# hvasbath/beat

Measured on AMD Instinct MI355X. Metric: SMC chain-steps/s (FFI seismic gfstacking 400 patches x 64 targets x 4096 samples), higher is better.
Workload: dtype f64

## Files before the change

### beat_amd/csrc/capi.cpp

```cpp
#include "kernels.hpp"

using namespace beatamd;

namespace {

int dev_alloc_copy(beatamd_ctx *ctx, const void *src, size_t bytes, void **dst)
{
    void *d = nullptr;
    hipError_t e = hipMalloc(&d, bytes ? bytes : 8);
    if (e != hipSuccess) {
        (void)hipGetLastError();
        set_error("hipMalloc(%zu bytes) failed: %s", bytes, hipGetErrorString(e));
        return BEATAMD_ENOMEM;
    }
    if (src && bytes) {
        e = hipMemcpyAsync(d, src, bytes, hipMemcpyDefault, ctx->stream);
        if (e == hipSuccess) e = hipStreamSynchronize(ctx->stream);
        if (e != hipSuccess) {
            (void)hipFree(d);
            set_error("hipMemcpy(%zu bytes) failed: %s", bytes, hipGetErrorString(e));
            return BEATAMD_EHIP;
        }
    }
    *dst = d;
// ... 21 lines not shown

#define ENTER(ctx)                                                    \
    BA_CHECK((ctx) != nullptr, BEATAMD_EINVAL, "ctx is NULL");        \
    BA_HIP(hipSetDevice((ctx)->device))

int wset_quad(beatamd_ctx *ctx, const WeightSet &w, int64_t C, const double *X, int64_t xs_c,
              int64_t xs_d, double *quad)
{
    if (w.kind == BEATAMD_W_SCALAR)
        return launch_scalar_quad(ctx, C, w.nd, w.M, X, xs_c, xs_d, w.w, quad);
    if (w.band >= 0 && w.wb && GfKnobs::get(gf_knobs(ctx).qf_band, 1) != 0)
        return launch_quadform_banded(ctx, w.wb, w.band, w.M, w.nd, C, X, xs_c, xs_d, quad, w.nd);
    QuadformCall q;
    q.A = w.w;
    q.a_stride = w.M * w.M;
    q.M = w.M;
    q.nd = w.nd;
    q.C = C;
    q.X = X;
    q.xs_c = xs_c;
    q.xs_d = xs_d;
    q.upper_tri = w.upper_tri;
    q.quad = quad;
    q.q_stride = w.nd;
    return launch_quadform(ctx, q);
}

struct LikeTail {
    LikeGroups grp;
    const int32_t *chain_bad = nullptr;
};

int ffi_logp_device(beatamd_ctx *ctx, FfiModel &m, int64_t C, const double *Q, double *LL,
                    LikeTail *tail = nullptr)
{
    const int64_t nllk = m.nllk();
    const int64_t np = m.layout.nparams;
    void *p = nullptr;
    LikeGroups grp;
    int64_t col = 0;

    ChainVec slips[4];
    for (int v = 0; v < m.layout.nvar; v++) slips[v] = ChainVec{Q, np, m.layout.slip_off[v]};

    int32_t *chain_bad = nullptr;
    if (!m.wavemaps.empty()) {
        BA_TRY(ctx->get_scratch(SL_CHAINBAD, (size_t)C * sizeof(int32_t), &p));
        chain_bad = (int32_t *)p;
        BA_HIP(hipMemsetAsync(chain_bad, 0, (size_t)C * sizeof(int32_t), ctx->stream));
    }

    if (!m.wavemaps.empty()) {
        BA_TRY(ctx->get_scratch(SL_ST0, (size_t)C * m.P * sizeof(double), &p));
        double *st0 = (double *)p;
        BA_TRY(launch_sweep_model(ctx, m, Q, C, st0, chain_bad));
        for (auto &wm : m.wavemaps) {
            WeightSet *ws = get_obj(ctx->wsets, wm.wset);
            BA_CHECK(ws, BEATAMD_EINVAL, "wavemap refers to a destroyed weight set");
            GfStackCall k;
            k.nvar = m.layout.nvar;
            for (int v = 0; v < k.nvar; v++) {
                k.libs[v] = get_obj(ctx->seislibs, wm.libs[v]);
                BA_CHECK(k.libs[v] && k.libs[v]->g, BEATAMD_EINVAL,
                         "wavemap refers to a destroyed / empty GF library");
                k.slips[v] = slips[v];
            }
            k.durations = ChainVec{Q, np, m.layout.durations_off};
            k.st.starttimes0 = st0;
            k.st.Q = Q;
            k.st.nparams = np;
            k.order_key[0] = ChainVec{Q, np, m.layout.nuc_strike_off};
            k.order_key[1] = ChainVec{Q, np, m.layout.nuc_dip_off};
            k.st.shift_off = wm.shift_off;
            k.st.nslot = wm.nslot; k.st.tslot = wm.tslot; k.st.slot_shift_off = wm.slot_shift_off;
            k.st.chain_bad = chain_bad;
            k.interp = wm.interp;
            k.f32 = wm.f32;
            k.C = C;
            k.data = wm.data;
            BA_TRY(ctx->get_scratch(SL_QUAD, (size_t)C * wm.T * sizeof(double), &p));
            double *quad = (double *)p;
            if (ws->kind == BEATAMD_W_SCALAR) {
                k.mode = GF_RESID_SCALAR;
                k.wscalar = ws->w;
                k.quad = quad;
                BA_TRY(launch_gfstack(ctx, k));
            } else if (ws->band == 1 && ws->wb && ws->M == wm.N && ws->nd == wm.T &&
                       GfKnobs::get(gf_knobs(ctx).qf_band, 1) != 0) {
                k.mode = GF_RESID_BAND1;
                k.band_w = ws->wb;
                k.quad = quad;
                BA_TRY(ctx->get_scratch(SL_RESID, (size_t)C * wm.T * wm.N * sizeof(double), &p));
                k.out = (double *)p;
                BA_TRY(launch_gfstack(ctx, k));
            } else {
                k.mode = GF_RESID_STORE;
                BA_TRY(ctx->get_scratch(SL_RESID, (size_t)C * wm.T * wm.N * sizeof(double), &p));
                k.out = (double *)p;
                BA_TRY(launch_gfstack(ctx, k));
                BA_TRY(wset_quad(ctx, *ws, C, k.out, wm.T * wm.N, wm.N, quad));
            }
            BA_TRY(launch_mvn_finish(ctx, C, wm.T, wm.N, quad, ws->slog, HpSrc{Q, np, wm.hp_off},
                                     LL + col, nllk));
            col += wm.T;
        }
        grp.end[grp.n++] = (int32_t)col;
    }
    if (m.has_geo) {
// ... 896 lines not shown
                double *z = (double *)p, *rs = nullptr;
                if (draw->df > 0) {
                    BA_TRY(ctx->get_scratch(SL_ROWSCALE, (size_t)C * 8, &p));
                    rs = (double *)p;
                }
                BA_TRY(launch_philox_normal(ctx, z, C, K, draw->seed, draw->step, draw->first_chain));
                BA_TRY(launch_philox_chain(ctx, C, draw->seed, draw->step, draw->first_chain, draw->df, lu, rs));
                GemmCall g;
                g.A = z; g.lda = K;
                g.B = (const double *)d_f; g.ldb = np; g.b_kn = 1;
                g.O = de; g.ldo = np;
                g.M = C; g.N = np; g.K = K;
                g.row_scale = rs;
                g.timer = "proposal";
                BA_TRY(launch_gemm_f64(ctx, g));
            } else {
                BA_TRY(launch_philox_univariate(ctx, de, C, np, draw->kind, (const double *)d_f, draw->seed,
                                                draw->step, draw->first_chain));
                BA_TRY(launch_philox_chain(ctx, C, draw->seed, draw->step, draw->first_chain, 0, lu, nullptr));
            }
            BA_TRY(launch_propose(ctx, C, np, (const double *)d_q0, de, (const double *)d_sc,
                                  (const double *)d_lo, (const double *)d_up, qprop, inb));
        }
        advance = true;
    } else {
        BA_TRY(stage_in(ctx, SL_IN1, delta, (size_t)C * np * 8, &d_de));
        BA_TRY(stage_in(ctx, SL_IN5, log_u, (size_t)C * 8, &d_lu));
        BA_TRY(launch_propose(ctx, C, np, (const double *)d_q0, (const double *)d_de,
                              (const double *)d_sc, (const double *)d_lo, (const double *)d_up, qprop,
                              inb));
    }
    LikeTail tail;
    const bool fold = nllk * 8 <= 48 * 1024;
    BA_TRY(ffi_logp_device(ctx, *m, C, qprop, lprop, fold ? &tail : nullptr));
    BA_TRY(launch_accept(ctx, C, np, nllk, (double *)d_q0, (double *)d_l0, qprop, lprop, inb,
                         (const double *)d_lu, beta, (const double *)d_be, (int32_t *)d_acc,
                         fold ? &tail.grp : nullptr, tail.chain_bad, acc_sum, n_acc, advance));
    return finish_out(ctx, recs, 3);
}

int beatamd_ffi_astep_batch(beatamd_ctx *ctx, int32_t model_id, int64_t C, double *Q0, double *L0,
                            const double *delta, const double *scaling, const double *lower,
                            const double *upper, const double *log_u, double beta,
                            int32_t *accepted)
{
    BA_CHECK(ctx != nullptr, BEATAMD_EINVAL, "ctx is NULL");
    return astep_impl(ctx, model_id, C, Q0, L0, delta, scaling, lower, upper, log_u, beta, nullptr,
                      accepted);
}

int beatamd_ffi_astep_batch_betas(beatamd_ctx *ctx, int32_t model_id, int64_t C, double *Q0,
                                  double *L0, const double *delta, const double *scaling,
                                  const double *lower, const double *upper, const double *log_u,
                                  const double *betas, int32_t *accepted)
{
    BA_CHECK(ctx != nullptr && betas != nullptr, BEATAMD_EINVAL, "ffi_astep_betas: NULL argument");
    return astep_impl(ctx, model_id, C, Q0, L0, delta, scaling, lower, upper, log_u, 1.0, betas,
                      accepted);
}

int beatamd_ffi_mstep_batch(beatamd_ctx *ctx, int32_t model_id, int64_t C, double *Q0, double *L0,
                            const double *factor, int64_t K, int32_t kind, int32_t df, uint64_t seed,
                            uint32_t step, int64_t first_chain, const double *scaling, const double *lower,
                            const double *upper, double beta, const double *betas, int32_t *accepted,
                            int32_t *accepted_sum, int64_t *n_accepted)
{
    BA_CHECK(ctx != nullptr, BEATAMD_EINVAL, "ctx is NULL");
// ... 551 lines not shown
```

### beat_amd/csrc/ctx.cpp

```cpp
#include "ctx.hpp"

#include <cstdlib>

namespace beatamd {

static thread_local char g_err[1024] = "";

void set_error(const char *fmt, ...)
{
    va_list ap;
    va_start(ap, fmt);
    vsnprintf(g_err, sizeof(g_err), fmt, ap);
    va_end(ap);
}

int DevBuf::reserve(size_t bytes)
{
    if (bytes <= cap) return BEATAMD_OK;
    size_t want = bytes + bytes / 4;
    if (p) {
        BA_HIP(hipDeviceSynchronize());
        BA_HIP(hipFree(p));
        p = nullptr;
        cap = 0;
// ... 147 lines not shown
        }
        if (st & ST_BAD_HYPO) {
            set_error("nucleation index outside the patch grid");
            return BEATAMD_EINVAL;
        }
        if (st & ST_BAD_COV) {
            set_error("Sample covariances contains Inf or NaN! Please try reducing the upper and lower bounds "
                      "of hyper parameters!");
            return BEATAMD_EBADCOV;
        }
        if (st & ST_NOT_PSD) {
            set_error("Matrix is not positive definite");
            return BEATAMD_ENOTPSD;
        }
        if (st & ST_BAD_SCALE) {
            set_error("PoissonProposal: a step width outside (0, 500] (or NaN): the draws of that parameter are NaN");
            return BEATAMD_EINVAL;
        }
    }
    return BEATAMD_OK;
}

namespace beatamd {

void GfKnobs::read_env()
{
    auto rd = [](const char *name) { const char *e = getenv(name); return e ? atoi(e) : KNOB_UNSET; };
    gf_kernel = rd("BEATAMD_GF_KERNEL"); gs_cg = rd("BEATAMD_GS_CG"); gs_ws = rd("BEATAMD_GS_WS"); gs_dma = rd("BEATAMD_GS_DMA");
    gs_nt = rd("BEATAMD_GS_NT"); ws_map = rd("BEATAMD_WS_MAP"); gs_pair = rd("BEATAMD_GS_PAIR"); gs_nthint = rd("BEATAMD_GS_NTHINT");
    gs_order = rd("BEATAMD_GS_ORDER"); gs_fit = rd("BEATAMD_GS_FIT"); gs_win = rd("BEATAMD_GS_WIN"); gf_tinv = rd("BEATAMD_GF_TINV");
    gs_tune = rd("BEATAMD_GS_TUNE"); gf_order = rd("BEATAMD_GF_ORDER"); gf_cgroup = rd("BEATAMD_GF_CGROUP"); gs_ml = rd("BEATAMD_GS_ML");
    gc_global = rd("BEATAMD_GC_GLOBAL"); gc_sort = rd("BEATAMD_GC_SORT"); gc_keys = rd("BEATAMD_GC_KEYS"); gc_bands = rd("BEATAMD_GC_BANDS"); gr_cap = rd("BEATAMD_GR_CAP");
    gr_pass_alloc = rd("BEATAMD_GR_PASS_ALLOC"); gr_var = rd("BEATAMD_GR_VAR"); sweep_v1 = rd("BEATAMD_SWEEP_V1"); qf_band = rd("BEATAMD_QF_BAND"); qf_fuse = rd("BEATAMD_QF_FUSE"); gf_split = rd("BEATAMD_GF_SPLIT"); gm_wave = rd("BEATAMD_GM_WAVE");
}

const GfKnobs &gf_knobs(beatamd_ctx *ctx)
{
    if (ctx->knobs_live) ctx->knobs.read_env();
    return ctx->knobs;
}

}

extern "C" {

const char *beatamd_last_error(void) { return g_err; }

int beatamd_version(void) { return BEATAMD_VERSION; }

int beatamd_ctx_create(int device, beatamd_ctx **out)
{
    BA_CHECK(out != nullptr, BEATAMD_EINVAL, "ctx_create: out is NULL");
    int ndev = 0;
    hipError_t e = hipGetDeviceCount(&ndev);
    if (e != hipSuccess || ndev == 0) {
        (void)hipGetLastError();
        set_error("no HIP device available (%s)", hipGetErrorString(e));
        return BEATAMD_EHIP;
    }
    BA_CHECK(device >= 0 && device < ndev, BEATAMD_EINVAL, "device %d out of range [0,%d)", device,
             ndev);
    BA_HIP(hipSetDevice(device));
    beatamd_ctx *c = new beatamd_ctx();
    c->device = device;
    BA_HIP(hipStreamCreateWithFlags(&c->own_stream, hipStreamNonBlocking));
    c->stream = c->own_stream;
// ... 159 lines not shown
```

### beat_amd/csrc/ctx.hpp

```cpp
#pragma once
#include <hip/hip_runtime.h>

#include <cstdarg>
#include <cstdint>
#include <cstdio>
#include <cstring>
#include <map>
#include <memory>
#include <string>
#include <vector>

#include "../../include/beat_amd.h"

namespace beatamd {

void set_error(const char *fmt, ...);

#define BA_HIP(expr)                                                                         \
    do {                                                                                     \
        hipError_t e_ = (expr);                                                              \
        if (e_ != hipSuccess) {                                                              \
            beatamd::set_error("%s:%d: %s -> %s", __FILE__, __LINE__, #expr,                 \
                               hipGetErrorString(e_));                                       \
            return BEATAMD_EHIP;                                                             \
// ... 80 lines not shown
struct GeomSources {
    int nsrc = 0;
    int32_t *kind = nullptr;
    int64_t *poff = nullptr;
    double *pfix = nullptr;
    double *east = nullptr, *north = nullptr, *los = nullptr;
    int64_t Nobs = 0;
    double nu = 0.25;
};

struct FfiModel {
    beatamd_ffi_layout layout;
    int32_t nsub = 0;
    std::vector<int32_t> ndip, nstrike, patch_off;
    std::vector<double> patch_size;
    int64_t P = 0;
    int32_t *d_ndip = nullptr, *d_nstrike = nullptr, *d_patch_off = nullptr;
    double *d_patch_size = nullptr;
    std::vector<Wavemap> wavemaps;
    bool has_geo = false;
    Geodetic geo;
    bool geo_is_geometry = false;
    GeomSources geom;
    int32_t lap = -1;
    int64_t nllk() const;
};

constexpr int KNOB_UNSET = -2147483647;
struct GfKnobs {
    int gf_kernel = KNOB_UNSET, gs_cg = KNOB_UNSET, gs_ws = KNOB_UNSET, gs_dma = KNOB_UNSET, gs_nt = KNOB_UNSET,
        ws_map = KNOB_UNSET, gs_pair = KNOB_UNSET, gs_nthint = KNOB_UNSET, gs_order = KNOB_UNSET, gs_fit = KNOB_UNSET,
        gs_win = KNOB_UNSET, gf_tinv = KNOB_UNSET, gs_tune = KNOB_UNSET, gf_order = KNOB_UNSET, gf_cgroup = KNOB_UNSET,
        gs_ml = KNOB_UNSET, gc_global = KNOB_UNSET, gc_sort = KNOB_UNSET, gc_keys = KNOB_UNSET, gc_bands = KNOB_UNSET, gr_cap = KNOB_UNSET,
        gr_pass_alloc = KNOB_UNSET, gr_var = KNOB_UNSET, sweep_v1 = KNOB_UNSET, qf_band = KNOB_UNSET, qf_fuse = KNOB_UNSET, gf_split = KNOB_UNSET, gm_wave = KNOB_UNSET;
    void read_env();
    static int get(int v, int dflt) { return v == KNOB_UNSET ? dflt : v; }
    static bool is(int v, int x) { return v != KNOB_UNSET && v == x; }
    static bool set(int v) { return v != KNOB_UNSET; }
};

struct KTimer {
    double total_ms = 0;
    int64_t n = 0;
    std::vector<std::pair<hipEvent_t, hipEvent_t>> pending;
};

}

struct beatamd_ctx {
    int device = 0;
    hipStream_t stream = nullptr, own_stream = nullptr;
    bool timing = false;
    std::map<std::string, beatamd::KTimer> timers;
    std::vector<hipEvent_t> event_pool;
    int *d_status = nullptr;
    std::vector<beatamd::DevBuf> scratch;
    std::vector<std::unique_ptr<beatamd::SeisLib>> seislibs;
    std::vector<std::unique_ptr<beatamd::GeoLib>> geolibs;
    std::vector<std::unique_ptr<beatamd::WeightSet>> wsets;
    std::vector<std::unique_ptr<beatamd::Laplacian>> laps;
    std::vector<std::unique_ptr<beatamd::FfiModel>> models;
    int num_cu = 256;
    char last_gf_kernel[96] = "";
    int64_t gs_ngtp = 0, gs_N = 0;
    double gs_trep = 1;
    int gs_nvar = 1;
    bool gs_has_passes = false;
// ... 19 lines not shown

namespace beatamd {

bool is_device_ptr(const void *p);
const GfKnobs &gf_knobs(beatamd_ctx *ctx);

struct Arg {
    beatamd_ctx *ctx;
    void *host = nullptr;
    void *dev = nullptr;
    size_t bytes = 0;
    bool out = false;
};

int stage_in(beatamd_ctx *ctx, int slot, const void *p, size_t bytes, const void **dev);
int stage_out(beatamd_ctx *ctx, int slot, void *p, size_t bytes, void **dev, Arg *rec,
              bool preload = false);
int finish_out(beatamd_ctx *ctx, Arg *recs, int n);

struct ScopedTimer {
    beatamd_ctx *c;
    const char *n;
    ScopedTimer(beatamd_ctx *ctx, const char *name) : c(ctx), n(name) { c->time_begin(n); }
    ~ScopedTimer() { c->time_end(n); }
};

enum Slot : int {
    SL_IN0 = 0, SL_IN1, SL_IN2, SL_IN3, SL_IN4, SL_IN5, SL_IN6, SL_IN7,
    SL_OUT0, SL_OUT1, SL_OUT2,
    SL_ROWOFF, SL_WEIGHTS, SL_ST0, SL_RESID, SL_PARTIAL, SL_PARTIAL2, SL_QUAD, SL_MU, SL_SLIPS,
    SL_QPROP, SL_LPROP, SL_MISC, SL_GS_UROWS, SL_GS_UCOUNT, SL_GS_SLOT, SL_GS_W, SL_GS_UMAX, SL_GS_USLOT,
    SL_CHAINBAD, SL_Z, SL_ROWSCALE, SL_CUM, SL_STAGE2, SL_WHITEN,
    SL_CHOL_A, SL_CHOL_X, SL_CHOL_D, SL_CHOL_T, SL_CHOL_L,
    SL_GC_ORDER, SL_GS_ORDER, SL_GC_STREAM, SL_GC_HDR, SL_GC_META, SL_DELTA, SL_LOGU, SL_EDGES, SL_TSLOT, SL_SPLIT, SL_COUNT
};

}
```

### beat_amd/csrc/gfshared.hip

```cpp
#include "kernels.hpp"

namespace beatamd {

constexpr int GS_NT_MAX = 64;
constexpr int GS_NTHINT_DEFAULT = 1;
constexpr int GS_WS_DEFAULT = 1;

struct GroupTabArgs {
    int nrow, nvar, CG;
    int64_t C, T, P, DS;
    const uint32_t *rowoff;
    const double *fac;
    ChainVec slips[4];
    int ucap, ustride;
    uint32_t *urows;
    uint32_t *uent;
    int nissue;
    int windowed;
    int depth;
    uint32_t *ucount;
    uint32_t *umax;
    uint16_t *slot;
    double *w;
    int64_t w_var_stride;
// ... 933 lines not shown
    const int64_t w_var_bytes = a.w_var_stride * 8;
    auto tab_slot = [&](int p) { return slot_base + (uint32_t)p * slot_step; };
    auto tab_w = [&](int p, int iv) {
        return w_base + (uint32_t)p * w_step + (nvar == 1 ? (int64_t)0 : (int64_t)iv * w_var_bytes);
    };
    auto fetch_tabs = [&](const char *ps, const char *pw) {
        asm("global_load_ushort %0, %1, %2" : "=v"(sl_n) : "v"(voff_s), "s"(ps));
        uint32_t voff_w;
        asm("v_lshlrev_b32 %1, 2, %2\n\t"
            "global_load_dwordx2 %0, %1, %3" : "=v"(wl_n), "=&v"(voff_w) : "v"(voff_s), "s"(pw));
    };
    auto row_address = [&](uint32_t base) {
        uint32_t x;
        asm("s_waitcnt vmcnt(0)\n\t"
            "v_lshl_add_u32 %0, %1, 6, %1\n\t"
            "v_lshl_add_u32 %0, %0, 3, %2" : "=&v"(x) : "v"(sl_n), "s"(base), "v"(wl_n));
        return x;
    };
    auto landed_weight = [&](uint32_t after) {
        double x;
        asm("v_mov_b64 %0, %1" : "=v"(x) : "v"(wl_n), "v"(after));
        return x;
    };
    static_assert(GS_PITCH == 65, "row_address multiplies by 65");
    constexpr int NG8 = GS_NT / 8;
    static_assert(NG8 == 8, "the read schedule below is written for 64-sample tiles");
    double ya[8], yb[8];
    int p1 = 0, iv1 = 0;
    advance(p1, iv1);
    int gbuf = 0;
    const int ring = NB * bufsz;
    double w;
    uint32_t xs;
    fetch_tabs(tab_slot(0), tab_w(0, 0));
    xs = row_address(lds0);
    w = landed_weight(xs);
    __builtin_amdgcn_sched_barrier(0);
    __builtin_amdgcn_s_barrier();
    __builtin_amdgcn_sched_barrier(0);
    lds_rd8_b64<0>(ya, xs, -1);
    lds_rd8_b64<64>(yb, xs, -1);
    __builtin_amdgcn_sched_barrier(0);
    fetch_tabs(tab_slot(p1), tab_w(p1, iv1));
    advance(p1, iv1);
    const char *ps_run = tab_slot(p1), *pw_run = tab_w(p1, iv1);
    int iv_run = iv1;
    const int64_t dw_next = (nvar == 1) ? (int64_t)w_step : w_var_bytes;
    const int64_t dw_wrap = (int64_t)w_step - (int64_t)(nvar - 1) * w_var_bytes;
#pragma clang loop unroll(disable)
    for (int s = 0; s < nsteps; s++) {
        int gnext = gbuf + bufsz;
        if (gnext == ring) gnext = 0;
        __builtin_amdgcn_sched_barrier(0);
#define BA_FMA8 \
    "v_fmac_f64 %0, %8, %16\n\tv_fmac_f64 %1, %9, %16\n\tv_fmac_f64 %2, %10, %16\n\tv_fmac_f64 %3, %11, %16\n\t" \
    "v_fmac_f64 %4, %12, %16\n\tv_fmac_f64 %5, %13, %16\n\tv_fmac_f64 %6, %14, %16\n\tv_fmac_f64 %7, %15, %16\n\t"
#define BA_RD8(OFF) \
    "ds_read_b64 %8, %17 offset:" #OFF "\n\tds_read_b64 %9, %17 offset:" #OFF "+8\n\t" \
    "ds_read_b64 %10, %17 offset:" #OFF "+16\n\tds_read_b64 %11, %17 offset:" #OFF "+24\n\t" \
    "ds_read_b64 %12, %17 offset:" #OFF "+32\n\tds_read_b64 %13, %17 offset:" #OFF "+40\n\t" \
    "ds_read_b64 %14, %17 offset:" #OFF "+48\n\tds_read_b64 %15, %17 offset:" #OFF "+56"
#define BA_ACC8(G) \
    "+v"(acc[G * 8]), "+v"(acc[G * 8 + 1]), "+v"(acc[G * 8 + 2]), "+v"(acc[G * 8 + 3]), "+v"(acc[G * 8 + 4]), \
        "+v"(acc[G * 8 + 5]), "+v"(acc[G * 8 + 6]), "+v"(acc[G * 8 + 7])
#define BA_Y8(Y) "+v"(Y[0]), "+v"(Y[1]), "+v"(Y[2]), "+v"(Y[3]), "+v"(Y[4]), "+v"(Y[5]), "+v"(Y[6]), "+v"(Y[7])
#define BA_FMA4A \
// ... 30 lines not shown
        asm(BA_FMA8
            "v_mov_b64 %16, %18\n\t" BA_RD8(64)
            : BA_ACC8(7), BA_Y8(yb), "+v"(w) : "v"(xs_n), "v"(wl_n));
        xs = xs_n;
        __builtin_amdgcn_sched_barrier(0);
#undef BA_GROUP
#undef BA_RD4B
#undef BA_RD4A
#undef BA_FMA4B
#undef BA_FMA4A
#undef BA_Y8
#undef BA_ACC8
#undef BA_RD8
#undef BA_FMA8
        fetch_tabs(ps_run, pw_run);
        {
            uint32_t ds;
            int64_t dw;
            asm("s_add_i32 %0, %0, 1\n\t"
                "s_cmp_eq_u32 %0, %3\n\t"
                "s_cselect_b32 %0, 0, %0\n\t"
                "s_cselect_b32 %1, %4, 0\n\t"
                "s_cselect_b64 %2, %5, %6"
                : "+s"(iv_run), "=&s"(ds), "=&s"(dw) : "s"(nvar), "s"(slot_step), "s"(dw_wrap), "s"(dw_next) : "scc");
            ps_run += ds;
            pw_run += dw;
        }
    }
    asm volatile("s_waitcnt vmcnt(0) lgkmcnt(0)"
                 : "+v"(ya[0]), "+v"(ya[1]), "+v"(ya[2]), "+v"(ya[3]), "+v"(ya[4]), "+v"(ya[5]), "+v"(ya[6]),
                   "+v"(ya[7]), "+v"(yb[0]), "+v"(yb[1]), "+v"(yb[2]), "+v"(yb[3]), "+v"(yb[4]), "+v"(yb[5]),
                   "+v"(yb[6]), "+v"(yb[7]), "+v"(sl_n), "+v"(wl_n));
    __builtin_amdgcn_sched_barrier(0);

    const bool live = (c < a.C);
    const int nvalid = (int)min((int64_t)GS_NT, N - n0);
    if (MODE == GF_STORE_SYN) {
        if (live) {
            double *o = a.out + (c * a.T + t) * N + n0;
#pragma unroll
            for (int i = 0; i < GS_NT; i++)
                if (i < nvalid) o[i] = acc[i];
        }
        return;
    }
    __builtin_amdgcn_s_barrier();
    if (tid < GS_NT) xbuf[tid] = (tid < nvalid) ? a.data[t * N + n0 + tid] : 0.0;
    if (MODE == GF_RESID_BAND1 && tid >= GS_NT && tid < 3 * GS_NT)
        xbuf[tid] = ((tid - GS_NT) >> 1) < nvalid ? a.band_w[(t * N + n0) * 2 + (tid - GS_NT)] : 0.0;
    __builtin_amdgcn_fence(__ATOMIC_RELEASE, "workgroup");
    __builtin_amdgcn_s_barrier();
    __builtin_amdgcn_fence(__ATOMIC_ACQUIRE, "workgroup");
    if (MODE == GF_RESID_BAND1) {
        const double *wbt = xbuf + GS_NT;
        const bool trace_end = n0 + nvalid == N;
        double q = 0.0, ri = xbuf[0] - acc[0];
        const double rfirst = ri;
#pragma unroll
        for (int i0 = 0; i0 < GS_NT; i0 += 8) {
#pragma unroll
            for (int i = i0; i < i0 + 8; i++) {
                if (i + 1 < nvalid) {
                    const double rn = xbuf[i + 1] - acc[i + 1];
                    double y = fma(wbt[2 * i], ri, 0.0);
                    y = fma(wbt[2 * i + 1], rn, y);
                    q = fma(y, y, q);
// ... 459 lines not shown
    uint32_t *utotal;
    uint32_t *ucount;
    uint32_t *uent;
    uint16_t *slot;
    double *w;
    int64_t w_var_stride;
    int64_t R;
};

__global__ void __launch_bounds__(256) k_ws_scan(const uint32_t *npass, uint32_t *voff, uint32_t *nv, int64_t P)
{
    __shared__ uint32_t part[256];
    const int tid = threadIdx.x;
    const int64_t gt = blockIdx.x;
    uint32_t run = 0;
    for (int64_t base = 0; base < P; base += 256) {
        const int64_t p = base + tid;
        const uint32_t x = p < P ? npass[gt * P + p] : 0u;
        part[tid] = x;
        __syncthreads();
        uint32_t before = 0, total = 0;
        for (int k = 0; k < 256; k++) {
            const uint32_t y = part[k];
            if (k < tid) before += y;
            total += y;
        }
        if (p < P) voff[gt * P + p] = run + before;
        run += total;
        __syncthreads();
    }
    if (tid == 0) nv[gt] = run;
}

constexpr int64_t WS_MAP_MAX = 16384;
template <int FILL, int MAP>
__global__ void __launch_bounds__(WS_CG) k_ws_tables(WsTabArgs a)
{
    extern __shared__ __attribute__((aligned(16))) uint16_t rowmap[];
    __shared__ __attribute__((aligned(16))) uint32_t vals[WS_CG];
    __shared__ __attribute__((aligned(16))) uint32_t firstv[WS_CG];
    __shared__ uint32_t lst[WS_CG];
    __shared__ uint32_t gm[WS_CG];
    __shared__ uint16_t slt[WS_CG];
    __shared__ uint8_t rk2i[WS_MAXPASS][128];
    __shared__ uint32_t wsum[WS_CG / 64 + 1];
    const int tid = threadIdx.x;
    const int lane = tid & 63, wv = tid >> 6;
    const int64_t gtp = xcd_items8(blockIdx.x, gridDim.x);
    const int64_t p = gtp % a.P;
    const int64_t gt = gtp / a.P;
    const int64_t t = gt % a.T;
    const int64_t g = gt / a.T;
    const int64_t pos_in_batch = g * WS_CG + tid;
    const bool live = pos_in_batch < a.C;
    const int64_t c = live ? (a.order ? (int64_t)a.order[pos_in_batch] : pos_in_batch) : 0;
    const uint32_t v = live ? a.rowoff[(c * a.T + t) * a.P + p] : 0xffffffffu;
    double sl[4] = {0.0, 0.0, 0.0, 0.0};
    if constexpr (FILL)
        for (int iv = 0; iv < a.nvar; iv++)
            if (live) sl[iv] = a.slips[iv].base[c * a.slips[iv].stride + a.slips[iv].off + (t % a.R) * a.P + p];
    gm[tid] = 0;
    uint32_t pos = 0, U = 0;
    bool first = false;
    if constexpr (MAP) {
        const uint32_t row0 = (uint32_t)((t * a.P + p) * a.DS);
        for (int64_t i = tid; i < a.DS; i += WS_CG) rowmap[i] = 0;
        __syncthreads();
        if (live) rowmap[v - row0] = 1;
        __syncthreads();
        uint32_t run = 0;
        for (int64_t base = 0; base < a.DS; base += WS_CG) {
            const int64_t i = base + tid;
            const uint32_t f = (i < a.DS) ? rowmap[i] : 0u;
            const uint64_t m = __ballot(f != 0);
            if (lane == 0) wsum[wv] = (uint32_t)__popcll(m);
            __syncthreads();
            uint32_t before = 0, total = 0;
            for (int q = 0; q < WS_CG / 64; q++) {
                const uint32_t x = wsum[q];
                if (q < wv) before += x;
                total += x;
            }
            if (f) {
                const uint32_t ps = run + before + (uint32_t)__popcll(m & ((1ull << lane) - 1ull));
                rowmap[i] = (uint16_t)ps;
                if constexpr (FILL) lst[ps] = row0 + (uint32_t)i;
            }
            run += total;
            __syncthreads();
        }
        U = run;
        if (live) pos = rowmap[v - row0];
    } else {
        vals[tid] = v;
        __syncthreads();
        first = live;
        {
            const uint4 *v4 = reinterpret_cast<const uint4 *>(vals);
            for (int k4 = 0; k4 < WS_CG / 4; k4++) {
                const uint4 x = v4[k4];
                const int k = 4 * k4;
                first = first && !((x.x == v && k < tid) || (x.y == v && k + 1 < tid) || (x.z == v && k + 2 < tid) ||
                                   (x.w == v && k + 3 < tid));
            }
        }
        firstv[tid] = first ? v : 0xffffffffu;
        {
            const uint64_t m = __ballot(first);
            if (lane == 0) wsum[wv] = (uint32_t)__popcll(m);
        }
        __syncthreads();
        if (live) {
            const uint4 *f4 = reinterpret_cast<const uint4 *>(firstv);
            for (int k4 = 0; k4 < WS_CG / 4; k4++) {
                const uint4 x = f4[k4];
                pos += (x.x < v) + (x.y < v) + (x.z < v) + (x.w < v);
            }
        }
        for (int q = 0; q < WS_CG / 64; q++) U += wsum[q];
    }
    const int npass = (int)((U + (uint32_t)a.cap - 1) / (uint32_t)a.cap);
    if constexpr (!FILL) {
        if (tid == 0) {
            a.npass[gtp] = (uint32_t)npass;
            a.utotal[gtp] = U;
        }
        return;
    }
    if (tid == 0) a.utotal[gtp] = U;
    const int per = ((int)U + npass - 1) / npass;
    if constexpr (!MAP) {
        if (first) lst[pos] = v;
    }
    if (live) atomicOr(&gm[pos], 1u << (tid >> 5));
    __syncthreads();
    const int mypass = live ? (int)pos / per : -1;
    if (wv < npass) {
        const int base = wv * per;
        const int n = min(per, (int)U - base);
        if (n <= 32) {
            if (lane < n) slt[base + lane] = (uint16_t)lane;
        } else {
            const int depth = a.cap / 32;
            const int r0 = lane, r1 = lane + 64;
            const uint32_t m0 = r0 < n ? gm[base + r0] : 0u, m1 = r1 < n ? gm[base + r1] : 0u;
            const int key0 = r0 < n ? ((__popc(m0) << 8) | (255 - r0)) : -1;
            const int key1 = r1 < n ? ((__popc(m1) << 8) | (255 - r1)) : -1;
            int rank0 = 0, rank1 = 0;
            for (int j = 0; j < n; j++) {
                const int kj = (__popc(gm[base + j]) << 8) | (255 - j);
                rank0 += kj > key0;
                rank1 += kj > key1;
            }
            if (r0 < n && rank0 < 32) slt[base + r0] = (uint16_t)rank0;
            if (r1 < n && rank1 < 32) slt[base + r1] = (uint16_t)rank1;
            if (r0 < n) rk2i[wv][rank0] = (uint8_t)r0;
            if (r1 < n) rk2i[wv][rank1] = (uint8_t)r1;
            wave_lds_fence();
            uint32_t wmask = 0;
            int wcnt = 0;
            if (lane < 32) {
                wmask = gm[base + rk2i[wv][lane]];
                wcnt = 1;
            }
            for (int rk = 32; rk < n; rk++) {
                const int ridx = (int)rk2i[wv][rk];
                const uint32_t mm = gm[base + ridx];
                int cost = (lane < 32 && wcnt < depth) ? ((__popc(wmask & mm) << 12) | (wcnt << 6) | lane) : 0x7fffffff;
#pragma unroll
                for (int off = 32; off > 0; off >>= 1) cost = min(cost, __shfl_xor(cost, off, 64));
                const int w = cost & 63;
                if (lane == w) {
                    slt[base + ridx] = (uint16_t)(w + 32 * wcnt);
                    wmask |= mm;
                    wcnt++;
                }
            }
        }
    }
    __syncthreads();
    const int64_t v0 = gt * a.vmax + (a.voff ? (int64_t)a.voff[gtp] : p);
    const uint16_t myslot = live ? slt[pos] : (uint16_t)0;
    constexpr int kstr = WS_USTRIDE / WS_LW;
    for (int k = 0; k < npass; k++) {
        const int64_t vs = v0 + k;
        const int base = k * per;
        const int n = min(per, (int)U - base);
        const bool mine = mypass == k;
        a.slot[vs * WS_CG + tid] = mine ? myslot : (uint16_t)a.cap;
        for (int iv = 0; iv < a.nvar; iv++) a.w[(int64_t)iv * a.w_var_stride + vs * WS_CG + tid] = mine ? sl[iv] : 0.0;
        if (tid == 0) a.ucount[vs] = (uint32_t)n;
        if (tid < WS_USTRIDE) {
            const int j = tid;
            uint32_t *e = a.uent + ((vs * WS_LW + (j % WS_LW)) * kstr + (j / WS_LW)) * 2;
            e[0] = lst[base + (j < n ? j : n - 1)];
            e[1] = j < n ? (uint32_t)slt[base + j] : 0u;
        }
    }
}

static int pick_group(int64_t C)
{
    const int cand[4] = {512, 256, 128, 64};
    const double cost[4] = {2.55, 1.5, 1.2, 1.0};
    int best = 64;
    double bestc = 1e300;
    for (int i = 0; i < 4; i++) {
        const double c = (double)((C + cand[i] - 1) / cand[i]) * cost[i];
        if (c < bestc - 1e-12) { bestc = c; best = cand[i]; }
    }
    return best;
}

static bool shared_fit(const GfStackCall &k, int cg, int *ucap_out)
{
    const SeisLib &L = *k.libs[0];
    const int nrow = k.interp == BEATAMD_MULTILINEAR ? 4 : 1;
    const int64_t DS = L.D * L.S;
    const int64_t ucap = std::min<int64_t>((int64_t)cg * nrow, DS);
    if (ws_wanted(k, cg)) {
        *ucap_out = (int)std::max<int64_t>(ucap, 2);
        return true;
    }
    if (2 * ucap * (GS_NT_MAX + 2) * 8 > 158 * 1024) return false;
    if (2 * DS * 4 + cg * 4 + 2048 > 60 * 1024) return false;
    *ucap_out = (int)std::max<int64_t>(ucap, 2);
    return true;
}
// ... 63 lines not shown
    const int64_t ngroups = (k.C + WS_CG - 1) / WS_CG;
    const int64_t GT = ngroups * Ttab, GTP = GT * L.P;
    const int64_t bound = std::min<int64_t>(WS_CG, L.D * L.S);
    const int cap = bound <= 32 ? 32 : bound <= 64 ? 64 : WS_CAP_MAX;
    const int maxpass = (int)((bound + cap - 1) / cap);
    const int64_t vmax = L.P * maxpass;
    void *p = nullptr;

    WsTabArgs ta;
    memset(&ta, 0, sizeof(ta));
    ta.nvar = k.nvar; ta.cap = cap;
    ta.C = k.C; ta.T = Ttab; ta.P = L.P; ta.DS = L.D * L.S; ta.vmax = vmax;
    ta.rowoff = rowoff;
    for (int v = 0; v < k.nvar; v++) ta.slips[v] = k.slips[v];
    ta.R = k.patch_split;
    if (ngroups > 1 && k.order_key[0].base && k.order_key[1].base && GfKnobs::get(kn.gc_global, 1) != 0)
        BA_TRY(launch_chain_members(ctx, k.C, k.order_key, WS_CG, ngroups, &ta.order, GfKnobs::get(kn.gc_global, 1) == 2));
    BA_TRY(ctx->get_scratch(SL_GS_UCOUNT, (size_t)(3 * GTP + GT) * sizeof(uint32_t), &p));
    ta.utotal = (uint32_t *)p;
    ta.npass = ta.utotal + GTP;
    uint32_t *voff = ta.npass + GTP, *nv = voff + GTP;
    const size_t nvs = (size_t)GT * vmax + 3;
    BA_TRY(ctx->get_scratch(SL_GS_UROWS, nvs * sizeof(uint32_t), &p));
    ta.ucount = (uint32_t *)p;
    BA_TRY(ctx->get_scratch(SL_GS_USLOT, nvs * WS_USTRIDE * 2 * sizeof(uint32_t), &p));
    ta.uent = (uint32_t *)p;
    BA_TRY(ctx->get_scratch(SL_GS_SLOT, nvs * WS_CG * sizeof(uint16_t), &p));
    ta.slot = (uint16_t *)p;
    ta.w_var_stride = (int64_t)GT * vmax * WS_CG;
    BA_TRY(ctx->get_scratch(SL_GS_W, ((size_t)ta.w_var_stride * k.nvar + (size_t)3 * WS_CG) * sizeof(double), &p));
    ta.w = (double *)p;
    {
        ScopedTimer tm(ctx, "grouptables");
        const bool map = ta.DS <= WS_MAP_MAX && !GfKnobs::is(kn.ws_map, 0);
        const size_t mlds = map ? (size_t)ta.DS * sizeof(uint16_t) : 0;
        if (maxpass > 1) {
            if (map) hipLaunchKernelGGL((k_ws_tables<0, 1>), dim3((unsigned)GTP), dim3(WS_CG), mlds, ctx->stream, ta);
            else hipLaunchKernelGGL((k_ws_tables<0, 0>), dim3((unsigned)GTP), dim3(WS_CG), 0, ctx->stream, ta);
            hipLaunchKernelGGL(k_ws_scan, dim3((unsigned)GT), dim3(256), 0, ctx->stream, ta.npass, voff, nv, L.P);
            ta.voff = voff;
        }
        if (map) hipLaunchKernelGGL((k_ws_tables<1, 1>), dim3((unsigned)GTP), dim3(WS_CG), mlds, ctx->stream, ta);
        else hipLaunchKernelGGL((k_ws_tables<1, 0>), dim3((unsigned)GTP), dim3(WS_CG), 0, ctx->stream, ta);
    }
    BA_HIP(hipGetLastError());

    GsArgs a;
    memset(&a, 0, sizeof(a));
    bool f32 = k.f32;
    const bool pair64 = GfKnobs::is(kn.gs_pair, 1);
    for (int v = 0; v < k.nvar; v++) {
        a.G[v] = k.libs[v]->g;
        a.G32[v] = k.libs[v]->g32;
        f32 = f32 && a.G32[v] != nullptr;
    }
    a.nvar = k.nvar; a.nrow = 1;
    a.C = k.C; a.T = L.T; a.P = L.P; a.N = L.N;
    a.Ttab = Ttab; a.rows_per_target = L.P * L.D * L.S;
    a.tslot = k.tslot;
    a.CG = WS_CG; a.ucap = cap; a.ustride = WS_USTRIDE;
    a.nt = 64; a.dma = 2; a.ws = 3;
    a.ngroups = ngroups;
    a.ntile = (int)((L.N + 63) / 64);
    a.nv = maxpass > 1 ? nv : nullptr;
    a.vmax = vmax;
    a.order = ta.order;
// ... 230 lines not shown
```

### beat_amd/csrc/gfstack.hip

```cpp
#include <cstdlib>
#include <cstring>

#include "kernels.hpp"

namespace beatamd {

struct TabArgs {
    int interp;
    int64_t C, T, P, D, S;
    double st_min, st_dt, du_min, du_dt;
    ChainVec durations;
    StartTimeSrc st;
    uint32_t *rowoff;
    double *fac;
    int *status;
    int64_t R;
};

__device__ __forceinline__ int to_int16(double x) { return (int)(int16_t)(long long)x; }

__device__ __forceinline__ bool wrap_index(int &i, int n)
{
    if (i < 0) i += n;
    return i >= 0 && i < n;
// ... 407 lines not shown
            double s_ = 0.0;
            for (int k = 0; k < ntile; k++) {
                s_ += tsum[k];
                if (k + 1 < ntile) {
                    const int last = k * 64 + 63;
                    double y = fma(w[2 * last], sq[last], 0.0);
                    y = fma(w[2 * last + 1], sq[last + 1], y);
                    s_ = fma(y, y, s_);
                }
            }
            quad[ct] = s_;
        }
        return;
    }
    if (n < ntile) {
        double q = 0.0;
        const int hi = (int)min((int64_t)64, N - (int64_t)n * 64);
        for (int i = 0; i < hi; i++) q = fma(sq[n * 64 + i], sq[n * 64 + i], q);
        tsum[n] = q;
    }
    __syncthreads();
    if (n == 0) {
        double s_ = 0.0;
        for (int k = 0; k < ntile; k++) s_ += tsum[k];
        quad[ct] = s_;
    }
}

static int launch_gfstack_split(beatamd_ctx *ctx, const GfStackCall &call, int R)
{
    const SeisLib &L = *call.libs[0];
    SeisLib views[4];
    GfStackCall v = call;
    for (int i = 0; i < call.nvar; i++) {
        views[i] = *call.libs[i];
        views[i].T = L.T * R;
        views[i].P = L.P / R;
        v.libs[i] = &views[i];
    }
    v.patch_split = R;
    v.mode = GF_STORE_SYN;
    void *p = nullptr;
    BA_TRY(ctx->get_scratch(SL_SPLIT, (size_t)call.C * L.T * R * L.N * sizeof(double), &p));
    double *part = (double *)p;
    v.out = part;
    v.quad = nullptr; v.data = nullptr; v.wscalar = nullptr; v.band_w = nullptr;
    BA_TRY(launch_gfstack_impl(ctx, v));
    for (int i = 0; i < call.nvar; i++) { views[i].g = nullptr; views[i].g32 = nullptr; }
    {
        const size_t n0 = strlen(ctx->gf_plan);
        snprintf(ctx->gf_plan + n0, sizeof(ctx->gf_plan) - n0, "; %lld-sample traces: patches stacked in %d ranges of %lld "
                 "(%lld walks instead of %lld), partial synthetics summed in range order", (long long)L.N, R, (long long)(L.P / R),
                 (long long)(L.T * R * ((L.N + 63) / 64)), (long long)(L.T * ((L.N + 63) / 64)));
    }
    const dim3 grid((unsigned)(call.C * L.T));
    BA_CHECK(call.C * L.T < (int64_t)0x7fffffff, BEATAMD_EINVAL, "gfstack: batch too large");
    ScopedTimer tm(ctx, "gfcombine");
    switch (call.mode) {
    case GF_STORE_SYN:
        hipLaunchKernelGGL(k_split_combine<GF_STORE_SYN>, grid, dim3(256), 0, ctx->stream, part, call.C, L.T, L.N, R, call.data,
                           call.wscalar, call.out, call.quad, (const double *)nullptr);
        break;
    case GF_RESID_SCALAR:
        hipLaunchKernelGGL(k_split_combine<GF_RESID_SCALAR>, grid, dim3(256), 0, ctx->stream, part, call.C, L.T, L.N, R, call.data,
                           call.wscalar, call.out, call.quad, (const double *)nullptr);
        break;
// ... 223 lines not shown
```

### beat_amd/csrc/kernels.hpp

```cpp
#pragma once
#include <algorithm>

#include "ctx.hpp"

namespace beatamd {

int launch_sweep_explicit(beatamd_ctx *ctx, const double *slow, double h, const int32_t *hi,
                          const int32_t *hj, int ni, int nj, int64_t C, double *out);
int launch_sweep_model(beatamd_ctx *ctx, const FfiModel &m, const double *Q, int64_t C,
                       double *starttimes0, int32_t *chain_bad);

struct StartTimeSrc {
    const double *explicit_st = nullptr;
    const double *starttimes0 = nullptr;
    const double *Q = nullptr;
    int64_t nparams = 0;
    const int64_t *shift_off = nullptr;
    int32_t nslot = 0;
    const int32_t *tslot = nullptr;
    const int64_t *slot_shift_off = nullptr;
    int32_t *chain_bad = nullptr;
};

struct ChainVec {
// ... 8 lines not shown
    const int64_t r = b & 63;
    return (b & ~(int64_t)63) + (r & 7) * 8 + (r >> 3);
}
#endif

int gf_patch_ranges(int64_t T, int64_t P, int64_t N, int num_cu);

enum GfMode : int {
    GF_STORE_SYN = 0,
    GF_RESID_SCALAR = 1,
    GF_RESID_STORE = 2,
    GF_RESID_BAND1 = 3
};

struct GfStackCall {
    const SeisLib *libs[4] = {nullptr, nullptr, nullptr, nullptr};
    int nvar = 1;
    ChainVec slips[4];
    ChainVec durations;
    StartTimeSrc st;
    int interp = 0;
    int64_t C = 0;
    int mode = GF_STORE_SYN;
    const double *data = nullptr;
    const double *wscalar = nullptr;
    double *out = nullptr;
    double *quad = nullptr;
    const double *band_w = nullptr;
    bool f32 = false;
    ChainVec order_key[2];
    int patch_split = 1;
    const GfKnobs *knobs = nullptr;
    const int32_t *tslot = nullptr;
};
int launch_gfstack(beatamd_ctx *ctx, const GfStackCall &call);
int launch_sum_tiles(beatamd_ctx *ctx, const double *partial, int64_t n, int ntile, double *quad,
                     const int *guard = nullptr, int want = 0);
int launch_sum_tiles_band1(beatamd_ctx *ctx, const double *partial, const double *edges, const double *band_w, int64_t C,
                           int64_t T, int64_t N, int ntile, int NT, double *quad, const int *guard = nullptr, int want = 0);
int launch_round_to_f32(beatamd_ctx *ctx, double *g, float *g32, int64_t n);
bool gfstack_shared_applicable(const GfStackCall &call, int *cg, int *ucap);
int gfstack_shared_candidates(const GfStackCall &call, int *cgs, int *ucaps);
int launch_gfstack_shared(beatamd_ctx *ctx, const GfStackCall &call, const uint32_t *rowoff,
                          const double *fac, int CG, int ucap, int64_t Ttab);

int launch_chain_members(beatamd_ctx *ctx, int64_t C, const ChainVec key[2], int64_t cg, int64_t ngroups, const uint32_t **members,
                         int strips = 0);
bool gfstack_ml_applicable(const GfStackCall &call);
int launch_gfstack_ml(beatamd_ctx *ctx, const GfStackCall &call, const uint32_t *rowoff,
                      const double *fac, int64_t Ttab, const int **ovf);

struct QuadformCall {
    const double *A = nullptr;
    int64_t a_stride = 0;
    int64_t M = 0, nd = 0, C = 0;
    const double *X = nullptr;
    int64_t xs_c = 0, xs_d = 0;
    int upper_tri = 0;
    double *quad = nullptr;
    int64_t q_stride = 0;
};
int launch_quadform(beatamd_ctx *ctx, const QuadformCall &call);
constexpr int QF_BAND_LIMIT = 16;
int launch_band_detect(beatamd_ctx *ctx, const double *A, int64_t nd, int64_t M, void *scratch, int64_t *band_host,
                       double *dropped_rel_host);
int launch_band_pack(beatamd_ctx *ctx, const double *A, int64_t nd, int64_t M, int64_t band, double *wb);
// ... 115 lines not shown
```

### beat_amd/csrc/logp.hip

```cpp
#include "kernels.hpp"

namespace beatamd {

#define LOG_2PI 1.8378770664093453

__device__ __forceinline__ double hp_value(const HpSrc &h, int64_t c, int64_t d)
{
    return h.base[c * h.stride + (h.offs ? h.offs[d] : d)];
}

__global__ void __launch_bounds__(256) k_mvn_finish(int64_t C, int64_t nd, int64_t M,
                                                   const double *quad, const double *slog,
                                                   HpSrc hp, double *logpts, int64_t ld)
{
    const int64_t i = (int64_t)blockIdx.x * 256 + threadIdx.x;
    if (i >= C * nd) return;
    const int64_t c = i / nd, d = i - c * nd;
    const double h = hp_value(hp, c, d);
    const double norm = (double)(int16_t)M * (2 * h + LOG_2PI);
    logpts[c * ld + d] = (-0.5) * (slog[d] + norm + (1 / exp(h * 2)) * quad[i]);
}

int launch_mvn_finish(beatamd_ctx *ctx, int64_t C, int64_t nd, int64_t M, const double *quad,
                      const double *slog, HpSrc hp, double *logpts, int64_t ld)
// ... 292 lines not shown
        const double q = Q0[c * nparams + k] + d;
        Qprop[c * nparams + k] = q;
        if (!(q >= lower[k] && q <= upper[k])) ok = 0;
    }
    if (!ok) s_ok = 0;
    __syncthreads();
    if (!s_ok)
        for (int64_t k = threadIdx.x; k < nparams; k += 256)
            Qprop[c * nparams + k] = Q0[c * nparams + k];
    if (threadIdx.x == 0) inbounds[c] = s_ok;
}

int launch_propose(beatamd_ctx *ctx, int64_t C, int64_t nparams, const double *Q0,
                   const double *delta, const double *scaling, const double *lower,
                   const double *upper, double *Qprop, int32_t *inbounds)
{
    if (C == 0) return BEATAMD_OK;
    hipLaunchKernelGGL(k_propose, dim3((unsigned)C), dim3(256), 0, ctx->stream, C, nparams, Q0,
                       delta, scaling, lower, upper, Qprop, inbounds);
    BA_HIP(hipGetLastError());
    return BEATAMD_OK;
}

__global__ void __launch_bounds__(256) k_accept(int64_t C, int64_t nparams, int64_t nllk,
                                               double *Q0, double *L0, const double *Qprop,
                                               double *Lprop, const int32_t *inbounds,
                                               const double *log_u, double beta,
                                               const double *betas, int32_t *accepted, LikeGroups grp,
                                               const int32_t *chain_bad, int32_t *acc_sum,
                                               unsigned long long *n_acc, uint32_t *step_dev)
{
    extern __shared__ __attribute__((aligned(16))) double s_l[];
    const int64_t c = blockIdx.x;
    double lp;
    if (grp.n > 0) {
        for (int64_t k = threadIdx.x; k < nllk - 1; k += 256) s_l[k] = Lprop[c * nllk + k];
        __syncthreads();
        if (threadIdx.x == 0) {
            double total = 0.0;
            int k = 0;
            for (int g = 0; g < grp.n; g++) {
                double s = 0.0;
                for (; k < grp.end[g]; k++) s += s_l[k];
                total += s;
            }
            if (chain_bad && chain_bad[c]) total = __builtin_nan("");
            s_l[nllk - 1] = total;
            Lprop[c * nllk + nllk - 1] = total;
        }
        __syncthreads();
        lp = s_l[nllk - 1];
    } else {
        lp = Lprop[c * nllk + nllk - 1];
    }
    const double b = betas ? betas[c] : beta;
    const double mr = b * (lp - L0[c * nllk + nllk - 1]);
    const bool acc = inbounds[c] && isfinite(mr) && (log_u[c] < mr);
    if (acc) {
        for (int64_t k = threadIdx.x; k < nparams; k += 256) Q0[c * nparams + k] = Qprop[c * nparams + k];
        __syncthreads();
        if (grp.n > 0) {
            for (int64_t k = threadIdx.x; k < nllk; k += 256) L0[c * nllk + k] = s_l[k];
        } else {
            for (int64_t k = threadIdx.x; k < nllk; k += 256) L0[c * nllk + k] = Lprop[c * nllk + k];
        }
    }
    if (threadIdx.x == 0) {
        accepted[c] = acc ? 1 : 0;
        if (acc_sum && acc) acc_sum[c] += 1;
        if (n_acc && acc) atomicAdd(n_acc, 1ull);
        if (step_dev && c == 0) *step_dev += 1u;
    }
}

int launch_accept(beatamd_ctx *ctx, int64_t C, int64_t nparams, int64_t nllk, double *Q0,
                  double *L0, const double *Qprop, double *Lprop, const int32_t *inbounds,
                  const double *log_u, double beta, const double *betas, int32_t *accepted,
                  const LikeGroups *grp, const int32_t *chain_bad, int32_t *acc_sum, int64_t *n_acc,
                  bool advance_step)
{
    if (C == 0) return BEATAMD_OK;
    LikeGroups g;
    if (grp) g = *grp;
    const size_t lds = grp ? (size_t)nllk * sizeof(double) : 0;
    BA_CHECK(lds <= 48 * 1024, BEATAMD_EINVAL, "accept: likelihood vector of %lld entries", (long long)nllk);
    ScopedTimer tm(ctx, "astep");
    hipLaunchKernelGGL(k_accept, dim3((unsigned)C), dim3(256), lds, ctx->stream, C, nparams, nllk,
                       Q0, L0, Qprop, Lprop, inbounds, log_u, beta, betas, accepted, g, chain_bad, acc_sum,
                       (unsigned long long *)n_acc, advance_step ? ctx->step_dev : nullptr);
    BA_HIP(hipGetLastError());
// ... 60 lines not shown
```

Before: 80240.

## Skip GF stacking for out-of-bounds proposal chains via compacted chain order

Adds a pack kernel that compacts the per-group chain order, keeping only chains whose proposal is in bounds, so the group-table and stacking kernels treat out-of-bounds chains as empty slots. Wavefronts with no live chain just hit the barriers and skip the stacking loop, and the accept kernel returns early for rejected-by-bounds chains. It is enabled by default through a new knob. The gain depends on the fraction of out-of-bounds proposals, and it costs an extra pack launch plus edge-case handling for groups with zero live chains.

```diff
diff --git a/beat_amd/csrc/capi.cpp b/beat_amd/csrc/capi.cpp
--- a/beat_amd/csrc/capi.cpp
+++ b/beat_amd/csrc/capi.cpp
@@ -77,7 +77,7 @@
 };
 
 int ffi_logp_device(beatamd_ctx *ctx, FfiModel &m, int64_t C, const double *Q, double *LL,
-                    LikeTail *tail = nullptr)
+                    LikeTail *tail = nullptr, const int32_t *active = nullptr)
 {
     const int64_t nllk = m.nllk();
     const int64_t np = m.layout.nparams;
@@ -119,6 +119,7 @@
             k.st.shift_off = wm.shift_off;
             k.st.nslot = wm.nslot; k.st.tslot = wm.tslot; k.st.slot_shift_off = wm.slot_shift_off;
             k.st.chain_bad = chain_bad;
+            k.active = active;
             k.interp = wm.interp;
             k.f32 = wm.f32;
             k.C = C;
@@ -1081,7 +1082,8 @@
     }
     LikeTail tail;
     const bool fold = nllk * 8 <= 48 * 1024;
-    BA_TRY(ffi_logp_device(ctx, *m, C, qprop, lprop, fold ? &tail : nullptr));
+    const int32_t *active = GfKnobs::get(gf_knobs(ctx).skip_parked, 1) != 0 ? inb : nullptr;
+    BA_TRY(ffi_logp_device(ctx, *m, C, qprop, lprop, fold ? &tail : nullptr, active));
     BA_TRY(launch_accept(ctx, C, np, nllk, (double *)d_q0, (double *)d_l0, qprop, lprop, inb,
                          (const double *)d_lu, beta, (const double *)d_be, (int32_t *)d_acc,
                          fold ? &tail.grp : nullptr, tail.chain_bad, acc_sum, n_acc, advance));
diff --git a/beat_amd/csrc/ctx.cpp b/beat_amd/csrc/ctx.cpp
--- a/beat_amd/csrc/ctx.cpp
+++ b/beat_amd/csrc/ctx.cpp
@@ -203,6 +203,7 @@
     gs_tune = rd("BEATAMD_GS_TUNE"); gf_order = rd("BEATAMD_GF_ORDER"); gf_cgroup = rd("BEATAMD_GF_CGROUP"); gs_ml = rd("BEATAMD_GS_ML");
     gc_global = rd("BEATAMD_GC_GLOBAL"); gc_sort = rd("BEATAMD_GC_SORT"); gc_keys = rd("BEATAMD_GC_KEYS"); gc_bands = rd("BEATAMD_GC_BANDS"); gr_cap = rd("BEATAMD_GR_CAP");
     gr_pass_alloc = rd("BEATAMD_GR_PASS_ALLOC"); gr_var = rd("BEATAMD_GR_VAR"); sweep_v1 = rd("BEATAMD_SWEEP_V1"); qf_band = rd("BEATAMD_QF_BAND"); qf_fuse = rd("BEATAMD_QF_FUSE"); gf_split = rd("BEATAMD_GF_SPLIT"); gm_wave = rd("BEATAMD_GM_WAVE");
+    skip_parked = rd("BEATAMD_SKIP_PARKED");
 }
 
 const GfKnobs &gf_knobs(beatamd_ctx *ctx)
diff --git a/beat_amd/csrc/ctx.hpp b/beat_amd/csrc/ctx.hpp
--- a/beat_amd/csrc/ctx.hpp
+++ b/beat_amd/csrc/ctx.hpp
@@ -136,7 +136,8 @@
         ws_map = KNOB_UNSET, gs_pair = KNOB_UNSET, gs_nthint = KNOB_UNSET, gs_order = KNOB_UNSET, gs_fit = KNOB_UNSET,
         gs_win = KNOB_UNSET, gf_tinv = KNOB_UNSET, gs_tune = KNOB_UNSET, gf_order = KNOB_UNSET, gf_cgroup = KNOB_UNSET,
         gs_ml = KNOB_UNSET, gc_global = KNOB_UNSET, gc_sort = KNOB_UNSET, gc_keys = KNOB_UNSET, gc_bands = KNOB_UNSET, gr_cap = KNOB_UNSET,
-        gr_pass_alloc = KNOB_UNSET, gr_var = KNOB_UNSET, sweep_v1 = KNOB_UNSET, qf_band = KNOB_UNSET, qf_fuse = KNOB_UNSET, gf_split = KNOB_UNSET, gm_wave = KNOB_UNSET;
+        gr_pass_alloc = KNOB_UNSET, gr_var = KNOB_UNSET, sweep_v1 = KNOB_UNSET, qf_band = KNOB_UNSET, qf_fuse = KNOB_UNSET, gf_split = KNOB_UNSET, gm_wave = KNOB_UNSET,
+        skip_parked = KNOB_UNSET;
     void read_env();
     static int get(int v, int dflt) { return v == KNOB_UNSET ? dflt : v; }
     static bool is(int v, int x) { return v != KNOB_UNSET && v == x; }
@@ -222,7 +223,7 @@
     SL_QPROP, SL_LPROP, SL_MISC, SL_GS_UROWS, SL_GS_UCOUNT, SL_GS_SLOT, SL_GS_W, SL_GS_UMAX, SL_GS_USLOT,
     SL_CHAINBAD, SL_Z, SL_ROWSCALE, SL_CUM, SL_STAGE2, SL_WHITEN,
     SL_CHOL_A, SL_CHOL_X, SL_CHOL_D, SL_CHOL_T, SL_CHOL_L,
-    SL_GC_ORDER, SL_GS_ORDER, SL_GC_STREAM, SL_GC_HDR, SL_GC_META, SL_DELTA, SL_LOGU, SL_EDGES, SL_TSLOT, SL_SPLIT, SL_COUNT
+    SL_GC_ORDER, SL_GS_ORDER, SL_GC_STREAM, SL_GC_HDR, SL_GC_META, SL_DELTA, SL_LOGU, SL_EDGES, SL_TSLOT, SL_SPLIT, SL_WS_PACK, SL_COUNT
 };
 
 }
diff --git a/beat_amd/csrc/gfshared.hip b/beat_amd/csrc/gfshared.hip
--- a/beat_amd/csrc/gfshared.hip
+++ b/beat_amd/csrc/gfshared.hip
@@ -989,6 +989,9 @@
     const int ring = NB * bufsz;
     double w;
     uint32_t xs;
+    if (__ballot(c < a.C) == 0) {
+        for (int s = 0; s <= nsteps; s++) __builtin_amdgcn_s_barrier();
+    } else {
     fetch_tabs(tab_slot(0), tab_w(0, 0));
     xs = row_address(lds0);
     w = landed_weight(xs);
@@ -1085,6 +1088,7 @@
                    "+v"(ya[7]), "+v"(yb[0]), "+v"(yb[1]), "+v"(yb[2]), "+v"(yb[3]), "+v"(yb[4]), "+v"(yb[5]),
                    "+v"(yb[6]), "+v"(yb[7]), "+v"(sl_n), "+v"(wl_n));
     __builtin_amdgcn_sched_barrier(0);
+    }
 
     const bool live = (c < a.C);
     const int nvalid = (int)min((int64_t)GS_NT, N - n0);
@@ -1610,6 +1614,28 @@
     if (tid == 0) nv[gt] = run;
 }
 
+__global__ void __launch_bounds__(WS_CG) k_ws_pack(const uint32_t *order, const int32_t *active, int64_t C, uint32_t *out)
+{
+    __shared__ uint32_t wsum[WS_CG / 64];
+    const int tid = threadIdx.x;
+    const int lane = tid & 63, wv = tid >> 6;
+    const int64_t pos = (int64_t)blockIdx.x * WS_CG + tid;
+    const uint32_t c = order ? order[pos] : (pos < C ? (uint32_t)pos : 0xffffffffu);
+    const bool on = c != 0xffffffffu && (int64_t)c < C && active[c] != 0;
+    const uint64_t m = __ballot(on);
+    if (lane == 0) wsum[wv] = (uint32_t)__popcll(m);
+    __syncthreads();
+    uint32_t before = 0, total = 0;
+    for (int q = 0; q < WS_CG / 64; q++) {
+        const uint32_t x = wsum[q];
+        if (q < wv) before += x;
+        total += x;
+    }
+    uint32_t *o = out + (int64_t)blockIdx.x * WS_CG;
+    if (on) o[before + (uint32_t)__popcll(m & ((1ull << lane) - 1ull))] = c;
+    if ((uint32_t)tid >= total) o[tid] = 0xffffffffu;
+}
+
 constexpr int64_t WS_MAP_MAX = 16384;
 template <int FILL, int MAP>
 __global__ void __launch_bounds__(WS_CG) k_ws_tables(WsTabArgs a)
@@ -1630,8 +1656,9 @@
     const int64_t t = gt % a.T;
     const int64_t g = gt / a.T;
     const int64_t pos_in_batch = g * WS_CG + tid;
-    const bool live = pos_in_batch < a.C;
-    const int64_t c = live ? (a.order ? (int64_t)a.order[pos_in_batch] : pos_in_batch) : 0;
+    const uint32_t oc = a.order ? a.order[pos_in_batch] : (uint32_t)pos_in_batch;
+    const bool live = pos_in_batch < a.C && oc != 0xffffffffu;
+    const int64_t c = live ? (int64_t)oc : 0;
     const uint32_t v = live ? a.rowoff[(c * a.T + t) * a.P + p] : 0xffffffffu;
     double sl[4] = {0.0, 0.0, 0.0, 0.0};
     if constexpr (FILL)
@@ -1697,7 +1724,7 @@
         }
         for (int q = 0; q < WS_CG / 64; q++) U += wsum[q];
     }
-    const int npass = (int)((U + (uint32_t)a.cap - 1) / (uint32_t)a.cap);
+    const int npass = U == 0 ? 1 : (int)((U + (uint32_t)a.cap - 1) / (uint32_t)a.cap);
     if constexpr (!FILL) {
         if (tid == 0) {
             a.npass[gtp] = (uint32_t)npass;
@@ -1706,7 +1733,7 @@
         return;
     }
     if (tid == 0) a.utotal[gtp] = U;
-    const int per = ((int)U + npass - 1) / npass;
+    const int per = U == 0 ? 1 : ((int)U + npass - 1) / npass;
     if constexpr (!MAP) {
         if (first) lst[pos] = v;
     }
@@ -1771,7 +1798,7 @@
         if (tid < WS_USTRIDE) {
             const int j = tid;
             uint32_t *e = a.uent + ((vs * WS_LW + (j % WS_LW)) * kstr + (j / WS_LW)) * 2;
-            e[0] = lst[base + (j < n ? j : n - 1)];
+            e[0] = n > 0 ? lst[base + (j < n ? j : n - 1)] : 0u;
             e[1] = j < n ? (uint32_t)slt[base + j] : 0u;
         }
     }
@@ -1901,6 +1928,11 @@
     ta.w = (double *)p;
     {
         ScopedTimer tm(ctx, "grouptables");
+        if (k.active) {
+            BA_TRY(ctx->get_scratch(SL_WS_PACK, (size_t)ngroups * WS_CG * sizeof(uint32_t), &p));
+            hipLaunchKernelGGL(k_ws_pack, dim3((unsigned)ngroups), dim3(WS_CG), 0, ctx->stream, ta.order, k.active, k.C, (uint32_t *)p);
+            ta.order = (const uint32_t *)p;
+        }
         const bool map = ta.DS <= WS_MAP_MAX && !GfKnobs::is(kn.ws_map, 0);
         const size_t mlds = map ? (size_t)ta.DS * sizeof(uint16_t) : 0;
         if (maxpass > 1) {
diff --git a/beat_amd/csrc/gfstack.hip b/beat_amd/csrc/gfstack.hip
--- a/beat_amd/csrc/gfstack.hip
+++ b/beat_amd/csrc/gfstack.hip
@@ -463,6 +463,7 @@
     const SeisLib &L = *call.libs[0];
     SeisLib views[4];
     GfStackCall v = call;
+    v.active = nullptr;
     for (int i = 0; i < call.nvar; i++) {
         views[i] = *call.libs[i];
         views[i].T = L.T * R;
diff --git a/beat_amd/csrc/kernels.hpp b/beat_amd/csrc/kernels.hpp
--- a/beat_amd/csrc/kernels.hpp
+++ b/beat_amd/csrc/kernels.hpp
@@ -64,6 +64,7 @@
     int patch_split = 1;
     const GfKnobs *knobs = nullptr;
     const int32_t *tslot = nullptr;
+    const int32_t *active = nullptr;
 };
 int launch_gfstack(beatamd_ctx *ctx, const GfStackCall &call);
 int launch_sum_tiles(beatamd_ctx *ctx, const double *partial, int64_t n, int ntile, double *quad,
diff --git a/beat_amd/csrc/logp.hip b/beat_amd/csrc/logp.hip
--- a/beat_amd/csrc/logp.hip
+++ b/beat_amd/csrc/logp.hip
@@ -348,6 +348,13 @@
 {
     extern __shared__ __attribute__((aligned(16))) double s_l[];
     const int64_t c = blockIdx.x;
+    if (!inbounds[c]) {
+        if (threadIdx.x == 0) {
+            accepted[c] = 0;
+            if (step_dev && c == 0) *step_dev += 1u;
+        }
+        return;
+    }
     double lp;
     if (grp.n > 0) {
         for (int64_t k = threadIdx.x; k < nllk - 1; k += 256) s_l[k] = Lprop[c * nllk + k];
@@ -371,7 +378,7 @@
     }
     const double b = betas ? betas[c] : beta;
     const double mr = b * (lp - L0[c * nllk + nllk - 1]);
-    const bool acc = inbounds[c] && isfinite(mr) && (log_u[c] < mr);
+    const bool acc = isfinite(mr) && (log_u[c] < mr);
     if (acc) {
         for (int64_t k = threadIdx.x; k < nparams; k += 256) Q0[c * nparams + k] = Qprop[c * nparams + k];
         __syncthreads();
```

Result: faster. 90770, median of 6 (+13.1%).
